# psmyth94/mamba-clip

Hardware: AMD Instinct MI355X
Metric: image-text pairs/sec (whole node) + selective_scan HBM GB/s (higher is better)
Workload: dtype bf16; 1 GPU; C2: ViT-B/16 image + Mamba-130M text, contrastive train step (fwd+bwd+AdamW), amp_bf16; model=vit_b16-mamba130m, global_batch=256, per_gpu_batch=256, seq_len=77, image_size=224, input=resident, step_launch=eager, parallelism=dp1, library_gemm_selection=tunableop-file

## Files before the change

### include/mc_gemm.h

```cpp
#ifndef MAMBA_CLIP_AMD_MC_GEMM_H
#define MAMBA_CLIP_AMD_MC_GEMM_H

#include <stddef.h>
#include <stdint.h>

#include "mc_scan.h"

#ifdef __cplusplus
extern "C" {
#endif

#define MC_WGRAD_TOKEN_MAJOR 0
#define MC_WGRAD_FEATURE_MAJOR 1

typedef struct mc_wgrad_params {
  int32_t M, N, T;
  int32_t dtype;
  int32_t a_layout, b_layout;
  const void* A;
  int64_t lda;
  const void* B;
  int64_t ldb;
  float* C;
  int64_t ldc;
  int32_t splits;
  int32_t reserved;
  void* workspace;
  size_t workspace_bytes;
} mc_wgrad_params;

size_t mc_gemm_wgrad_workspace_bytes(const mc_wgrad_params* p);
int mc_gemm_wgrad(const mc_wgrad_params* p, void* stream);

#define MC_LINEAR_EPI_NONE 0
#define MC_LINEAR_EPI_BIAS 1
#define MC_LINEAR_EPI_BIAS_GELU 2
#define MC_LINEAR_EPI_GELU_GRAD 3

typedef struct mc_linear_params {
  int32_t rows, cols, K;
  int32_t dtype;
  int32_t epilogue;
  int32_t reserved;
  const void* X; int64_t ldx;
  const void* W; int64_t ldw;
  void* Y; int64_t ldy;
  void* Y2; int64_t ldy2;
  const void* bias;
  const void* H; int64_t ldh;
  float* colsum;
  void* workspace;
  size_t workspace_bytes;
} mc_linear_params;

size_t mc_linear_workspace_bytes(const mc_linear_params* p);
int mc_linear(const mc_linear_params* p, void* stream);

int mc_gemm_small_k(int32_t M, int32_t K, int32_t T, int32_t dtype, const void* W, int64_t ldw, const void* X,
                    int64_t ldx, void* Y, int64_t ldy, void* stream);

int mc_gemm_skinny_m(int32_t M, int32_t K, int32_t T, int32_t dtype, const void* W, int64_t ldw, const void* X,
                     int64_t ldx, void* Y, int64_t ldy, void* stream);

#ifdef __cplusplus
}
#endif

#endif
```

### mamba-clip_amd/csrc/ops.hip

```cpp
#include <algorithm>

#include "mc_common.h"
#include "../../include/mc_ops.h"

namespace mc {
namespace ops {

constexpr int kMaxVec = 8;

template <int V>
__device__ __forceinline__ void ld_f32v(const float* __restrict__ p, float (&v)[V]) {
#pragma unroll
  for (int e4 = 0; e4 < V; e4 += 4) {
    const float4 q = *reinterpret_cast<const float4*>(p + e4);
    v[e4] = q.x; v[e4 + 1] = q.y; v[e4 + 2] = q.z; v[e4 + 3] = q.w;
  }
}
template <int V>
__device__ __forceinline__ void st_f32v(float* __restrict__ p, const float (&v)[V]) {
#pragma unroll
  for (int e4 = 0; e4 < V; e4 += 4)
    *reinterpret_cast<float4*>(p + e4) = make_float4(v[e4], v[e4 + 1], v[e4 + 2], v[e4 + 3]);
}

// ... 1337 lines not shown
__global__ __launch_bounds__(256) void adamw_kernel(const mc_adamw_chunk* __restrict__ chunks,
                                                    const mc_adamw_tensor* __restrict__ tensors, const mc_adamw_hyper hy) {
  const mc_adamw_chunk c = chunks[blockIdx.x];
  const mc_adamw_tensor t = tensors[c.tensor];
  const mc_adamw_group h = hy.group[c.group];
  float* __restrict__ p = t.p + c.off;
  float* __restrict__ m = t.m + c.off;
  float* __restrict__ v = t.v + c.off;
  const float* __restrict__ g = t.g + c.off;
  const bool vec = ((reinterpret_cast<uintptr_t>(p) | reinterpret_cast<uintptr_t>(m) | reinterpret_cast<uintptr_t>(v) |
                     reinterpret_cast<uintptr_t>(g)) & 15) == 0;
  const int64_t n4 = vec ? c.n / 4 : 0;
  for (int64_t i = threadIdx.x; i < n4; i += 256) {
    float4 pp = reinterpret_cast<float4*>(p)[i], mm = reinterpret_cast<float4*>(m)[i];
    float4 vv = reinterpret_cast<float4*>(v)[i];
    const float4 gg = reinterpret_cast<const float4*>(g)[i];
    adamw_elem(pp.x, mm.x, vv.x, gg.x, h);
    adamw_elem(pp.y, mm.y, vv.y, gg.y, h);
    adamw_elem(pp.z, mm.z, vv.z, gg.z, h);
    adamw_elem(pp.w, mm.w, vv.w, gg.w, h);
    reinterpret_cast<float4*>(p)[i] = pp;
    reinterpret_cast<float4*>(m)[i] = mm;
    reinterpret_cast<float4*>(v)[i] = vv;
  }
  for (int64_t i = 4 * n4 + threadIdx.x; i < c.n; i += 256) {
    float pp = p[i], mm = m[i], vv = v[i];
    adamw_elem(pp, mm, vv, g[i], h);
    p[i] = pp;
    m[i] = mm;
    v[i] = vv;
  }
}
}

extern "C" int mc_adamw_step(int32_t n_chunks, const mc_adamw_chunk* chunks, const mc_adamw_tensor* tensors,
                             const mc_adamw_hyper* hyper, void* stream) {
  MC_CHECK(n_chunks >= 0 && hyper, MC_ERR_INVALID, "mc_adamw_step: bad arguments");
  MC_CHECK(hyper->n_groups >= 1 && hyper->n_groups <= MC_ADAMW_MAX_GROUPS, MC_ERR_INVALID,
           "mc_adamw_step: n_groups %d (1..%d)", hyper->n_groups, MC_ADAMW_MAX_GROUPS);
  if (n_chunks == 0) return MC_OK;
  MC_CHECK(chunks && tensors, MC_ERR_INVALID, "mc_adamw_step: null chunk / tensor table");
  hipLaunchKernelGGL(adamw_kernel, dim3(n_chunks), dim3(256), 0, (hipStream_t)stream, chunks, tensors, *hyper);
  return check_launch("mc_adamw_step");
}

namespace {
template <bool kVec>
__global__ __launch_bounds__(256) void sum_slabs_kernel(int s, int64_t n, const float* __restrict__ src, int64_t stride,
                                                        float* __restrict__ dst) {
  const int64_t i0 = ((int64_t)blockIdx.x * 256 + threadIdx.x) * (kVec ? 4 : 1);
  if (i0 >= n) return;
  if constexpr (kVec) {
    float4 acc = *reinterpret_cast<const float4*>(src + i0);
    for (int k = 1; k < s; ++k) {
      const float4 v = *reinterpret_cast<const float4*>(src + (int64_t)k * stride + i0);
      acc.x += v.x; acc.y += v.y; acc.z += v.z; acc.w += v.w;
    }
    *reinterpret_cast<float4*>(dst + i0) = acc;
  } else {
    float acc = src[i0];
    for (int k = 1; k < s; ++k) acc += src[(int64_t)k * stride + i0];
    dst[i0] = acc;
  }
}
}

extern "C" int mc_sum_slabs(int32_t s, int64_t n, const float* src, int64_t slab_stride, float* dst, void* stream) {
  MC_CHECK(s >= 1 && n >= 0 && slab_stride >= n, MC_ERR_SHAPE, "mc_sum_slabs: bad shape (s %d, n %lld, stride %lld)", s,
           (long long)n, (long long)slab_stride);
  if (n == 0) return MC_OK;
  MC_CHECK(src && dst, MC_ERR_INVALID, "mc_sum_slabs: null pointer");
  const bool vec = n % 4 == 0 && slab_stride % 4 == 0 && aligned16(src) && aligned16(dst);
  const int64_t items = vec ? n / 4 : n;
  const dim3 grid((unsigned)((items + 255) / 256));
  if (vec) hipLaunchKernelGGL(sum_slabs_kernel<true>, grid, dim3(256), 0, (hipStream_t)stream, s, n, src, slab_stride, dst);
  else hipLaunchKernelGGL(sum_slabs_kernel<false>, grid, dim3(256), 0, (hipStream_t)stream, s, n, src, slab_stride, dst);
  return check_launch("mc_sum_slabs");
}

static int colsum_slices(int rows) { return std::max(1, std::min(kGradSlices, (rows + 31) / 32)); }

extern "C" size_t mc_colsum_workspace_bytes(int32_t rows, int32_t cols) {
  return (size_t)colsum_slices(std::max(rows, 0)) * (size_t)std::max(cols, 0) * sizeof(float);
}

extern "C" int mc_colsum(int32_t rows, int32_t cols, int32_t dtype, const void* x, int64_t ld, float* out,
                         void* workspace, size_t workspace_bytes, void* stream) {
  MC_CHECK(dtype >= MC_DTYPE_F32 && dtype <= MC_DTYPE_F16, MC_ERR_DTYPE, "mc_colsum: bad dtype");
  MC_CHECK(rows >= 0 && cols >= 0 && ld >= cols, MC_ERR_SHAPE, "mc_colsum: bad shape (rows %d, cols %d, ld %lld)",
           rows, cols, (long long)ld);
  hipStream_t s = (hipStream_t)stream;
  if (cols == 0) return MC_OK;
  MC_CHECK(out, MC_ERR_INVALID, "mc_colsum: null output");
  if (rows == 0) {
    (void)hipMemsetAsync(out, 0, (size_t)cols * 4, s);
    return check_launch("mc_colsum");
  }
  MC_CHECK(x && workspace && workspace_bytes >= mc_colsum_workspace_bytes(rows, cols), MC_ERR_WORKSPACE,
           "mc_colsum: x and a workspace of mc_colsum_workspace_bytes required");
  float* part = reinterpret_cast<float*>(workspace);
  const int ns = colsum_slices(rows);
  const int V = dtype == MC_DTYPE_F32 ? 4 : 8;
  const bool vec = cols % V == 0 && ld % V == 0 && aligned16(x);
  MC_DISPATCH_T(dtype, {
    if (vec)
      hipLaunchKernelGGL((colsum_rows_kernel<T, ElemTraits<T>::kVec>), dim3((unsigned)((cols / V + 63) / 64), ns),
                         dim3(256), 0, s, rows, cols, (const T*)x, ld, part);
// ... 41 lines not shown
```

### mamba-clip_amd/mamba_clip_amd/_lib.py

```python
import ctypes
import os

_HERE = os.path.dirname(os.path.abspath(__file__))
LIB_PATH = os.environ.get("MAMBA_CLIP_AMD_LIB") or os.path.join(_HERE, "libmamba_clip_amd.so")

MC_DTYPE_F32, MC_DTYPE_BF16, MC_DTYPE_F16, MC_DTYPE_FP8_E4M3, MC_DTYPE_U8 = 0, 1, 2, 3, 4
MC_LAYOUT_NCHW, MC_LAYOUT_NHWC = 0, 1
MC_SCAN_CHUNK = 32
MC_SCAN_STATE_INTERVAL_FINE = 8
MC_SCAN_KERNEL_NONE, MC_SCAN_KERNEL_PAIR, MC_SCAN_KERNEL_GENERIC, MC_SCAN_KERNEL_DIRS = 0, 1, 2, 3
MC_GEMM_KERNEL_TILE, MC_GEMM_KERNEL_FP8_TILE, MC_GEMM_KERNEL_FP8_PANEL = 1, 2, 3
MC_SCAN_MAX_DSTATE = 32
MC_CAST_CHUNK = 16384

c_i32, c_i64, c_vp, c_fp = ctypes.c_int32, ctypes.c_int64, ctypes.c_void_p, ctypes.c_void_p


class ScanFwdParams(ctypes.Structure):
    _fields_ = [
        ("batch", c_i32), ("dim", c_i32), ("seqlen", c_i32), ("dstate", c_i32), ("n_groups", c_i32),
        ("itype", c_i32), ("wtype", c_i32), ("delta_softplus", c_i32),
        ("u_batch_stride", c_i64), ("u_dim_stride", c_i64),
        ("delta_batch_stride", c_i64), ("delta_dim_stride", c_i64),
        ("z_batch_stride", c_i64), ("z_dim_stride", c_i64),
# ... 170 lines not shown
class SS2DMergeBwdParams(ctypes.Structure):
    _fields_ = [
        ("fwd", SS2DMergeParams), ("dy", c_vp),
        ("dy_batch_stride", c_i64), ("dy_row_stride", c_i64), ("dy_col_stride", c_i64),
        ("dout", c_fp), ("dz", c_vp), ("dln_weight", c_fp), ("dln_bias", c_fp),
        ("workspace", c_vp), ("workspace_bytes", ctypes.c_size_t),
    ]


MC_WGRAD_TOKEN_MAJOR, MC_WGRAD_FEATURE_MAJOR = 0, 1


class WgradParams(ctypes.Structure):
    _fields_ = [
        ("M", c_i32), ("N", c_i32), ("T", c_i32), ("dtype", c_i32), ("a_layout", c_i32), ("b_layout", c_i32),
        ("A", c_vp), ("lda", c_i64), ("B", c_vp), ("ldb", c_i64), ("C", c_vp), ("ldc", c_i64),
        ("splits", c_i32), ("reserved", c_i32), ("workspace", c_vp), ("workspace_bytes", ctypes.c_size_t),
    ]


MC_LINEAR_EPI_NONE, MC_LINEAR_EPI_BIAS, MC_LINEAR_EPI_BIAS_GELU, MC_LINEAR_EPI_GELU_GRAD = 0, 1, 2, 3


class LinearParams(ctypes.Structure):
    _fields_ = [
        ("rows", c_i32), ("cols", c_i32), ("K", c_i32), ("dtype", c_i32), ("epilogue", c_i32), ("reserved", c_i32),
        ("X", c_vp), ("ldx", c_i64), ("W", c_vp), ("ldw", c_i64), ("Y", c_vp), ("ldy", c_i64),
        ("Y2", c_vp), ("ldy2", c_i64), ("bias", c_vp), ("H", c_vp), ("ldh", c_i64), ("colsum", c_vp),
        ("workspace", c_vp), ("workspace_bytes", ctypes.c_size_t),
    ]


class PatchInputParams(ctypes.Structure):
    _fields_ = [
        ("batch", c_i32), ("channels", c_i32), ("height", c_i32), ("width", c_i32), ("patch", c_i32),
        ("layout", c_i32), ("in_dtype", c_i32), ("out_dtype", c_i32),
        ("img", c_vp), ("scale", c_fp), ("shift", c_fp), ("out", c_vp),
    ]


SYMBOLS = {
    "mc_last_error": (ctypes.c_char_p, []),
    "mc_version": (ctypes.c_char_p, []),
    "mc_scan_n_chunks": (c_i32, [c_i32]),
    "mc_scan_n_states": (c_i32, [c_i32, c_i32]),
    "mc_scan_fwd_state_interval": (c_i32, [ctypes.POINTER(ScanFwdParams)]),
    "mc_scan_fwd_kernel": (c_i32, [ctypes.POINTER(ScanFwdParams)]),
    "mc_gemm_wgrad_workspace_bytes": (ctypes.c_size_t, [ctypes.POINTER(WgradParams)]),
    "mc_gemm_wgrad": (ctypes.c_int, [ctypes.POINTER(WgradParams), c_vp]),
    "mc_linear_workspace_bytes": (ctypes.c_size_t, [ctypes.POINTER(LinearParams)]),
    "mc_linear": (ctypes.c_int, [ctypes.POINTER(LinearParams), c_vp]),
    "mc_gemm_small_k": (ctypes.c_int, [c_i32, c_i32, c_i32, c_i32, c_vp, c_i64, c_vp, c_i64, c_vp, c_i64, c_vp]),
    "mc_gemm_skinny_m": (ctypes.c_int, [c_i32, c_i32, c_i32, c_i32, c_vp, c_i64, c_vp, c_i64, c_vp, c_i64, c_vp]),
    "mc_scan_bwd_kernel": (c_i32, [ctypes.POINTER(ScanBwdParams)]),
    "mc_scan_chunk_states_bytes": (ctypes.c_size_t, [c_i32, c_i32, c_i32, c_i32]),
    "mc_scan_fwd_workspace_bytes": (ctypes.c_size_t, [c_i32, c_i32, c_i32, c_i32]),
    "mc_scan_bwd_workspace_bytes": (ctypes.c_size_t, [c_i32, c_i32, c_i32, c_i32, c_i32]),
    "mc_scan_fwd": (ctypes.c_int, [ctypes.POINTER(ScanFwdParams), c_vp]),
    "mc_scan_bwd": (ctypes.c_int, [ctypes.POINTER(ScanBwdParams), c_vp]),
    "mc_gemm_nt": (ctypes.c_int, [ctypes.POINTER(GemmNTParams), c_vp]),
    "mc_gemm_nt_kernel": (c_i32, [ctypes.POINTER(GemmNTParams)]),
    "mc_quant_rows_fp8": (ctypes.c_int, [c_i32, c_i32, c_i32, c_vp, c_i64, c_vp, c_i64, c_fp, c_vp]),
    "mc_ce_stats": (ctypes.c_int, [c_i32, c_i32, c_fp, c_i64, c_i32, c_i64, c_fp, c_fp, ctypes.c_float, c_fp,
                                   c_vp, ctypes.c_size_t, c_vp]),
    "mc_ce_stats_workspace_bytes": (ctypes.c_size_t, [c_i32, c_i32, c_i32]),
    "mc_ce_grad": (ctypes.c_int, [c_i32, c_i32, c_fp, c_i64, c_fp, c_i64, ctypes.c_float, c_fp, c_i64,
                                  ctypes.c_float, c_fp, c_i32, c_vp, c_i64, c_fp, c_fp, c_vp, ctypes.c_size_t, c_vp]),
    "mc_ce_grad_workspace_bytes": (ctypes.c_size_t, [c_i32, c_i32]),
    "mc_ce_fused_fwd": (ctypes.c_int, [ctypes.POINTER(CEFusedParams), c_vp]),
    "mc_ce_fused_fwd_workspace_bytes": (ctypes.c_size_t, [c_i32, c_i32, c_i32]),
    "mc_ce_fused_grad": (ctypes.c_int, [ctypes.POINTER(CEFusedParams), c_vp]),
    "mc_ce_fused_grad_workspace_bytes": (ctypes.c_size_t, [c_i32, c_i32]),
    "mc_add_rmsnorm_fwd": (ctypes.c_int, [c_i32, c_i32, c_i32, c_vp, c_fp, c_fp, ctypes.c_float, c_vp, c_fp, c_fp,
                                          c_vp]),
    "mc_add_rmsnorm_bwd": (ctypes.c_int, [c_i32, c_i32, c_i32, c_vp, c_fp, c_fp, c_fp, c_fp, c_vp, c_fp, c_fp, c_vp,
                                          ctypes.c_size_t, c_vp]),
    "mc_add_rmsnorm_bwd_workspace_bytes": (ctypes.c_size_t, [c_i32, c_i32]),
    "mc_add_layernorm_fwd": (ctypes.c_int, [c_i32, c_i32, c_i32, c_vp, c_vp, c_fp, c_fp, ctypes.c_float, c_vp, c_vp,
                                            c_fp, c_fp, c_vp]),
    "mc_add_layernorm_bwd": (ctypes.c_int, [c_i32, c_i32, c_i32, c_vp, c_vp, c_vp, c_fp, c_fp, c_fp, c_vp, c_fp, c_fp,
                                            c_fp, c_vp, ctypes.c_size_t, c_vp]),
    "mc_add_layernorm_bwd_workspace_bytes": (ctypes.c_size_t, [c_i32, c_i32]),
    "mc_causal_conv1d_fwd": (ctypes.c_int, [c_i32, c_i32, c_i32, c_i32, c_i32, c_vp, c_i64, c_i64, c_fp, c_fp, c_i32,
                                            c_vp, c_i64, c_i64, c_vp]),
    "mc_causal_conv1d_bwd": (ctypes.c_int, [c_i32, c_i32, c_i32, c_i32, c_i32, c_vp, c_i64, c_i64, c_fp, c_fp, c_i32,
                                            c_vp, c_i64, c_i64, c_vp, c_i64, c_i64, c_fp, c_fp, c_vp,
                                            ctypes.c_size_t, c_vp]),
    "mc_causal_conv1d_bwd_workspace_bytes": (ctypes.c_size_t, [c_i32, c_i32, c_i32, c_i32]),
    "mc_patch_im2col": (ctypes.c_int, [c_i32, c_i32, c_i32, c_i32, c_i32, c_i32, c_vp, c_vp, c_vp]),
    "mc_grad_colsum_workspace_bytes": (ctypes.c_size_t, [c_i32, c_i32]),
    "mc_gelu_bwd": (ctypes.c_int, [c_i32, c_i32, c_i32, c_vp, c_i64, c_vp, c_i64, c_vp, c_i64, c_fp, c_vp,
                                   ctypes.c_size_t, c_vp]),
    "mc_qkv_grad_pack": (ctypes.c_int, [ctypes.POINTER(QkvPackParams), c_vp]),
    "mc_stream_copy": (ctypes.c_int, [c_vp, c_vp, ctypes.c_size_t, c_vp]),
    "mc_cast_f32_many": (ctypes.c_int, [c_i32, c_vp, c_vp, c_i32, c_vp]),
    "mc_cast_transpose_f32_many": (ctypes.c_int, [c_i32, c_vp, c_vp, c_i32, c_vp]),
    "mc_adamw_step": (ctypes.c_int, [c_i32, c_vp, c_vp, ctypes.POINTER(AdamWHyper), c_vp]),
    "mc_sum_slabs": (ctypes.c_int, [c_i32, c_i64, c_fp, c_i64, c_fp, c_vp]),
    "mc_colsum_workspace_bytes": (ctypes.c_size_t, [c_i32, c_i32]),
    "mc_colsum_fold": (ctypes.c_int, [c_i32, c_i32, c_fp, c_fp, c_vp]),
    "mc_colsum": (ctypes.c_int, [c_i32, c_i32, c_i32, c_vp, c_i64, c_fp, c_vp, ctypes.c_size_t, c_vp]),
    "mc_l2norm_fwd": (ctypes.c_int, [c_i32, c_i32, c_i32, c_vp, c_i64, ctypes.c_float, c_fp, c_i64, c_fp, c_vp]),
    "mc_l2norm_bwd": (ctypes.c_int, [c_i32, c_i32, c_i32, c_vp, c_i64, c_fp, ctypes.c_float, c_fp, c_i64, c_vp,
                                     c_i64, c_vp]),
    "mc_attn_fwd": (ctypes.c_int, [ctypes.POINTER(AttnFwdParams), c_vp]),
    "mc_attn_bwd": (ctypes.c_int, [ctypes.POINTER(AttnBwdParams), c_vp]),
# ... 58 lines not shown
```

### mamba-clip_amd/mamba_clip_amd/ops.py

```python
import ctypes
import os
import weakref

import torch

from . import _lib


def _ws(nbytes, device):
    return torch.empty(max(int(nbytes), 16), dtype=torch.uint8, device=device)


def gemm_nt(A, B, alpha=1.0, alpha_dev=None, out_dtype=torch.float32, scale_a=None, scale_b=None, out=None):
    lib = _lib.load()
    if A.dtype != B.dtype or A.dtype not in (torch.bfloat16, torch.float32, torch.float8_e4m3fn):
        raise RuntimeError("gemm_nt: A and B must both be bf16, both fp32 or both float8_e4m3fn")
    if A.stride(-1) != 1:
        A = A.contiguous()
    if B.stride(-1) != 1:
        B = B.contiguous()
    M, K = A.shape
    N, K2 = B.shape
    if K != K2:
        raise RuntimeError("gemm_nt: inner dimensions differ")
# ... 518 lines not shown
def patch_im2col(img, patch, out_dtype=None, mean=None, std=None):
    return PatchIm2colFn.apply(img, patch, out_dtype, mean, std)


def _split_factor(M, N, K):
    if N * K >= 2_000_000:
        s = 4
    elif N * K < 250_000 or M >= 40_000:
        s = 16
    else:
        s = 8
    while s > 1 and M % s:
        s //= 2
    return s


def _wgrad_layout(t, rows_are_tokens):
    st_tok, st_feat = (t.stride(0), t.stride(1)) if rows_are_tokens else (t.stride(1), t.stride(0))
    if st_feat == 1 and t.shape[1 if rows_are_tokens else 0] > 0:
        return _lib.MC_WGRAD_TOKEN_MAJOR, st_tok
    if st_tok == 1:
        return _lib.MC_WGRAD_FEATURE_MAJOR, st_feat
    return None


def wgrad_hip(G, X, splits=0):
    if not (G.is_cuda and G.dtype == X.dtype and G.dtype in (torch.bfloat16, torch.float16)):
        return None
    N, T = G.shape
    K = X.shape[1]
    la, lb = _wgrad_layout(G, False), _wgrad_layout(X, True)
    if la is None or lb is None or T % 64 or T == 0 or G.data_ptr() % 16 or X.data_ptr() % 16:
        return None
    if la[1] % 8 or lb[1] % 8 or (la[0] == _lib.MC_WGRAD_TOKEN_MAJOR and N % 8) or \
            (lb[0] == _lib.MC_WGRAD_TOKEN_MAJOR and K % 8):
        return None
    out = torch.empty(N, K, device=G.device, dtype=torch.float32)
    p = _lib.WgradParams()
    p.M, p.N, p.T, p.dtype = N, K, T, _lib.dtype_code(G.dtype)
    p.a_layout, p.lda, p.b_layout, p.ldb = la[0], la[1], lb[0], lb[1]
    p.A, p.B, p.C, p.ldc, p.splits = G.data_ptr(), X.data_ptr(), out.data_ptr(), K, int(splits)
    lib = _lib.load()
    ws_b = lib.mc_gemm_wgrad_workspace_bytes(ctypes.byref(p))
    ws = _ws(ws_b, G.device) if ws_b else None
    if ws is not None:
        p.workspace, p.workspace_bytes = ws.data_ptr(), ws_b
    _lib.check(lib.mc_gemm_wgrad(ctypes.byref(p), _lib.stream_handle(G.device)), "mc_gemm_wgrad")
    return out


WGRAD_HIP = os.environ.get("MAMBA_CLIP_AMD_WGRAD_HIP", "1") != "0"


def wgrad(G, X):
    N, M = G.shape
    K = X.shape[1]
    if WGRAD_HIP and G.is_cuda and M >= 8192 and min(N, K) >= 256:
        out = wgrad_hip(G, X)
        if out is not None:
            return out
    s = _split_factor(M, N, K) if (G.is_cuda and M >= 8192) else 1
    if s == 1:
        return torch.mm(G, X).float()
    Gs = G.unflatten(1, (s, M // s)).transpose(0, 1)
    Xs = X.unflatten(0, (s, M // s))
    part = torch.bmm(Gs, Xs, out_dtype=torch.float32).contiguous()
    out = torch.empty(N, K, device=part.device, dtype=torch.float32)
    _lib.check(_lib.load().mc_sum_slabs(s, N * K, part.data_ptr(), part.stride(0), out.data_ptr(),
                                        _lib.stream_handle(part.device)), "mc_sum_slabs")
    return out


def colsum(x):
    if x.stride(-1) != 1:
        x = x.contiguous()
    R, C = x.shape
    out = torch.empty(C, device=x.device, dtype=torch.float32)
    lib = _lib.load()
    ws_b = lib.mc_colsum_workspace_bytes(R, C)
    ws = _ws(ws_b, x.device)
    _lib.check(lib.mc_colsum(R, C, _lib.dtype_code(x.dtype), x.data_ptr(), x.stride(0), out.data_ptr(), ws.data_ptr(),
                             ws_b, _lib.stream_handle(x.device)), "mc_colsum")
    return out


class L2NormalizeFn(torch.autograd.Function):

    @staticmethod
    def forward(ctx, x, eps):
        x2 = x if x.stride(-1) == 1 else x.contiguous()
        R, C = x2.shape
        y = torch.empty(R, C, device=x.device, dtype=torch.float32)
        norm = torch.empty(R, device=x.device, dtype=torch.float32)
        _lib.check(_lib.load().mc_l2norm_fwd(R, C, _lib.dtype_code(x2.dtype), x2.data_ptr(), x2.stride(0), eps,
                                             y.data_ptr(), C, norm.data_ptr(), _lib.stream_handle(x.device)),
                   "mc_l2norm_fwd")
        ctx.save_for_backward(x2, norm)
        ctx.eps = eps
        return y

    @staticmethod
    def backward(ctx, g):
        x2, norm = ctx.saved_tensors
        g = g.float()
        if g.stride(-1) != 1:
            g = g.contiguous()
        R, C = x2.shape
        dx = torch.empty(R, C, device=x2.device, dtype=x2.dtype)
        _lib.check(_lib.load().mc_l2norm_bwd(R, C, _lib.dtype_code(x2.dtype), x2.data_ptr(), x2.stride(0),
                                             norm.data_ptr(), ctx.eps, g.data_ptr(), g.stride(0), dx.data_ptr(), C,
                                             _lib.stream_handle(x2.device)), "mc_l2norm_bwd")
        return dx, None

# ... 292 lines not shown
                db = pre[0]
            elif g2.is_cuda:
                db = colsum(g2)
            else:
                db = torch.sum(g2, 0, dtype=torch.float32)
        return dx, dw, db


def linear_sk(x, weight, bias=None):
    return LinearSK.apply(x, weight, bias)


SMALL_K_HIP = os.environ.get("MAMBA_CLIP_AMD_SMALL_K_HIP", "1") != "0"


def small_k_ok(wc, Xc):
    K = wc.shape[1]
    return (SMALL_K_HIP and Xc.is_cuda and wc.dtype == Xc.dtype and Xc.dtype in (torch.bfloat16, torch.float16)
            and K in (16, 32, 48, 64) and Xc.shape[1] % 8 == 0 and Xc.stride(1) == 1 and Xc.stride(0) % 8 == 0
            and Xc.data_ptr() % 16 == 0 and wc.stride(1) == 1 and wc.stride(0) % 4 == 0 and wc.data_ptr() % 8 == 0)


def gemm_small_k(wc, Xc):
    M, K = wc.shape
    T = Xc.shape[1]
    y = torch.empty(M, T, device=Xc.device, dtype=Xc.dtype)
    _lib.check(_lib.load().mc_gemm_small_k(M, K, T, _lib.dtype_code(Xc.dtype), wc.data_ptr(), wc.stride(0),
                                           Xc.data_ptr(), Xc.stride(0), y.data_ptr(), T,
                                           _lib.stream_handle(Xc.device)), "mc_gemm_small_k")
    return y


SKINNY_M_HIP = os.environ.get("MAMBA_CLIP_AMD_SKINNY_M_HIP", "0") == "1"


def skinny_m_ok(wc, Xc):
    M, K = wc.shape
    return (SKINNY_M_HIP and Xc.is_cuda and wc.dtype == Xc.dtype and Xc.dtype in (torch.bfloat16, torch.float16)
            and 0 < M <= 96 and K % 256 == 0 and Xc.shape[1] % 8 == 0 and Xc.stride(1) == 1
            and Xc.stride(0) % 8 == 0 and Xc.data_ptr() % 16 == 0 and wc.stride(1) == 1 and wc.stride(0) % 4 == 0
            and wc.data_ptr() % 8 == 0)


def gemm_skinny_m(wc, Xc):
    M, K = wc.shape
    T = Xc.shape[1]
    y = torch.empty(M, T, device=Xc.device, dtype=Xc.dtype)
    _lib.check(_lib.load().mc_gemm_skinny_m(M, K, T, _lib.dtype_code(Xc.dtype), wc.data_ptr(), wc.stride(0),
                                            Xc.data_ptr(), Xc.stride(0), y.data_ptr(), T,
                                            _lib.stream_handle(Xc.device)), "mc_gemm_skinny_m")
    return y


class WeightLeftMM(torch.autograd.Function):

    @staticmethod
    def forward(ctx, weight, X, handoff=None, out_slab=None):
        dt = _compute_dtype(X)
        wc, Xc = _wcast(weight, dt), X.to(dt)
        with torch.autocast("cuda", enabled=False):
            if small_k_ok(wc, Xc):
                y = gemm_small_k(wc, Xc)
            elif skinny_m_ok(wc, Xc):
                y = gemm_skinny_m(wc, Xc)
            else:
                y = torch.mm(wc, Xc)
        ctx.save_for_backward(wc, Xc)
        ctx.handoff = handoff
        ctx.out_slab = out_slab
        return y

    @staticmethod
    def backward(ctx, gy):
        wc, Xc = ctx.saved_tensors
        g = gy.to(wc.dtype)
        dw = dX = None
        if ctx.needs_input_grad[0]:
            dw = wgrad(g, Xc.t())
        acc = ctx.handoff.take() if ctx.handoff is not None else None
        if ctx.needs_input_grad[1]:
            accv = acc.transpose(0, 1) if (acc is not None and Xc.is_contiguous()) else None
            accv = accv.view(Xc.shape) if (accv is not None and accv.is_contiguous()
                                           and accv.numel() == Xc.numel()) else None
            if accv is not None:
                dX = accv
                dX.addmm_(wc.t(), g)
                acc = None
            elif Xc.stride(0) == 1 and Xc.stride(1) != 1:
                dX = torch.mm(g.t(), wc).t()
            elif ctx.out_slab is not None and acc is None and Xc.is_contiguous():
                slab, r0 = ctx.out_slab
                dX = slab.get()[r0:r0 + Xc.shape[0]]
                torch.mm(wc.t(), g, out=dX)
            else:
                dX = torch.mm(wc.t(), g)
            if acc is not None:
                dX = dX + acc.transpose(0, 1).reshape(Xc.shape)
        return dw, dX, None, None


def wleft_mm(weight, X, handoff=None, out_slab=None):
    return WeightLeftMM.apply(weight, X, handoff, out_slab)


def mixer_proj_ok(x_cm, rank, dstate):
    dt = _compute_dtype(x_cm)
    D, T = x_cm.shape
    return (x_cm.is_cuda and dt in (torch.bfloat16, torch.float16) and x_cm.stride(1) == 1 and D % 64 == 0
            and T % 8 == 0 and T > 0 and rank % 16 == 0 and 16 <= rank <= 96 and dstate == 16
            and x_cm.stride(0) % 8 == 0 and x_cm.data_ptr() % 16 == 0)


class MixerProjFn(torch.autograd.Function):

    @staticmethod
    def forward(ctx, x, w_x, w_dt, handoff):
        dt = _compute_dtype(x)
        lib = _lib.load()
        xc = x if x.dtype == dt else x.to(dt)
        wx, wdt = _wcast(w_x, dt).contiguous(), _wcast(w_dt, dt).contiguous()
        D, T = xc.shape
        P, R = wx.shape[0], wdt.shape[1]
        xd = torch.empty(P, T, device=xc.device, dtype=dt)
        delta = torch.empty(D, T, device=xc.device, dtype=dt)
        p = _lib.MixerProjParams()
        p.dim, p.tokens, p.rank, p.proj_rows, p.dtype = D, T, R, P, _lib.dtype_code(dt)
        p.x_ld, p.x_dbl_ld, p.delta_ld = xc.stride(0), T, T
        p.x, p.w_x, p.w_dt, p.x_dbl, p.delta = xc.data_ptr(), wx.data_ptr(), wdt.data_ptr(), xd.data_ptr(), delta.data_ptr()
        _lib.check(lib.mc_mixer_proj_fwd(ctypes.byref(p), _lib.stream_handle(xc.device)), "mc_mixer_proj_fwd")
        ctx.save_for_backward(xc, wx, wdt, xd)
        ctx.handoff = handoff
        return xd[R:P - 16], xd[P - 16:], delta

    @staticmethod
    def backward(ctx, g_b, g_c, g_delta):
        xc, wx, wdt, xd = ctx.saved_tensors
        lib = _lib.load()
        D, T = xc.shape
        P, R = wx.shape[0], wdt.shape[1]
# ... 575 lines not shown
```

Before: 3721 image-text pairs/sec.

## Add skinny-wgrad and small-K accumulate HIP kernels for Mamba x_proj backward

Adds a split-token MFMA wgrad kernel for weight gradients where one dimension is at most 48 rows, used in place of bmm plus slab-sum for the long-token skinny case. Also adds a small-K backward dX GEMM that fuses the accumulation into an existing buffer, replacing addmm_ when shapes qualify, and unrolls the slab-sum loop by eight to expose more loads in flight. These target the Mamba dt/B/C projection backward, where rocBLAS handles skinny shapes poorly. The cost is new custom kernels with their own edge-case handling, plus a workspace for the partial sums.

```diff
diff --git a/include/mc_gemm.h b/include/mc_gemm.h
--- a/include/mc_gemm.h
+++ b/include/mc_gemm.h
@@ -62,6 +62,13 @@
 int mc_gemm_skinny_m(int32_t M, int32_t K, int32_t T, int32_t dtype, const void* W, int64_t ldw, const void* X,
                      int64_t ldx, void* Y, int64_t ldy, void* stream);
 
+int mc_gemm_small_k_acc(int32_t M, int32_t K, int32_t T, int32_t dtype, const void* Wk, int64_t ldw, const void* X,
+                        int64_t ldx, const void* Z, int64_t ldz, void* Y, int64_t ldy, void* stream);
+
+size_t mc_wgrad_skinny_workspace_bytes(int32_t R, int32_t D, int32_t T);
+int mc_wgrad_skinny(int32_t R, int32_t D, int32_t T, int32_t dtype, const void* S, int64_t lds, const void* Wd,
+                    int64_t ldw, int32_t wide_major, float* C, void* workspace, size_t workspace_bytes, void* stream);
+
 #ifdef __cplusplus
 }
 #endif
diff --git a/mamba-clip_amd/csrc/gemm_skinny.hip b/mamba-clip_amd/csrc/gemm_skinny.hip
--- /dev/null
+++ b/mamba-clip_amd/csrc/gemm_skinny.hip
@@ -0,0 +1,312 @@
+#include <algorithm>
+#include <type_traits>
+
+#include "mc_common.h"
+#include "../../include/mc_gemm.h"
+
+extern "C" int mc_sum_slabs(int32_t s, int64_t n, const float* src, int64_t slab_stride, float* dst, void* stream);
+
+namespace mc {
+namespace skinny_wgrad {
+constexpr int kWD = 128;
+constexpr int kTok = 128;
+constexpr int kRow = 272;
+constexpr int kTargetWG = 256;
+constexpr int kPD = 4;
+
+typedef __bf16 bf16x8 __attribute__((ext_vector_type(8)));
+typedef _Float16 f16x8 __attribute__((ext_vector_type(8)));
+
+template <typename T>
+__device__ __forceinline__ f32x4 mfma32(const uint4& a, const uint4& b, const f32x4& c) {
+  if constexpr (std::is_same<T, bf16_t>::value)
+    return __builtin_amdgcn_mfma_f32_16x16x32_bf16(__builtin_bit_cast(bf16x8, a), __builtin_bit_cast(bf16x8, b), c, 0, 0, 0);
+  else
+    return __builtin_amdgcn_mfma_f32_16x16x32_f16(__builtin_bit_cast(f16x8, a), __builtin_bit_cast(f16x8, b), c, 0, 0, 0);
+}
+
+template <typename T, int NB>
+__global__ __launch_bounds__(256) void wgrad_skinny_kernel(int R, int D, int Tn, int chunks_per, int dblocks,
+                                                           const T* __restrict__ S, int64_t lds_,
+                                                           const T* __restrict__ Wd, int64_t ldw,
+                                                           float* __restrict__ P, int64_t slab, int wide_major) {
+  __shared__ __attribute__((aligned(16))) char sm[2][NB * 16 * kRow];
+  const int tid = threadIdx.x, lane = tid & 63, w = tid >> 6;
+  const int g = lane >> 4, i = lane & 15;
+  const int db = blockIdx.x % dblocks, rg = blockIdx.x / dblocks;
+  const int d0 = db * kWD + 32 * w;
+  const int nchunks = (Tn + kTok - 1) / kTok;
+  const int c0 = rg * chunks_per, c1 = min(nchunks, c0 + chunks_per);
+  int64_t wrow[2];
+#pragma unroll
+  for (int rb = 0; rb < 2; ++rb) wrow[rb] = (int64_t)min(d0 + 16 * rb + i, D - 1) * ldw;
+  struct Bundle { uint4 w[2][4]; uint4 s[NB]; };
+  Bundle q[kPD];
+  auto keep = [](bool ok, const uint4& v) __attribute__((always_inline)) {
+    return make_uint4(ok ? v.x : 0u, ok ? v.y : 0u, ok ? v.z : 0u, ok ? v.w : 0u);
+  };
+  const int sr = tid >> 4, st = (tid & 15) * 8;
+  auto load = [&](int c, Bundle& b) __attribute__((always_inline)) {
+    const int t0 = c * kTok;
+    const bool live = c < c1;
+#pragma unroll
+    for (int rb = 0; rb < 2; ++rb)
+#pragma unroll
+      for (int s = 0; s < 4; ++s) {
+        const int t = t0 + 32 * s + 8 * g;
+        b.w[rb][s] = ld16(Wd + ((live & (t < Tn)) ? wrow[rb] + t : (int64_t)0));
+      }
+#pragma unroll
+    for (int j = 0; j < NB; ++j) {
+      const int r = sr + 16 * j, t = t0 + st;
+      b.s[j] = ld16(S + ((live & (r < R) & (t < Tn)) ? (int64_t)r * lds_ + t : (int64_t)0));
+    }
+  };
+  f32x4 acc[2][NB];
+#pragma unroll
+  for (int rb = 0; rb < 2; ++rb)
+#pragma unroll
+    for (int nb = 0; nb < NB; ++nb) acc[rb][nb] = f32x4{0.f, 0.f, 0.f, 0.f};
+#pragma unroll
+  for (int d = 0; d < kPD; ++d) load(c0 + d, q[d]);
+  int c = c0;
+  auto step = [&](Bundle& b) __attribute__((always_inline)) {
+    char* img = sm[(c - c0) & 1];
+    const int t0 = c * kTok;
+#pragma unroll
+    for (int j = 0; j < NB; ++j)
+      *reinterpret_cast<uint4*>(img + (sr + 16 * j) * kRow + st * 2) = keep(sr + 16 * j < R && t0 + st < Tn, b.s[j]);
+    __syncthreads();
+    uint4 n[4][NB];
+#pragma unroll
+    for (int s = 0; s < 4; ++s)
+#pragma unroll
+      for (int nb = 0; nb < NB; ++nb)
+        n[s][nb] = *reinterpret_cast<const uint4*>(img + (16 * nb + i) * kRow + 64 * s + 16 * g);
+    __builtin_amdgcn_sched_barrier(0);
+#pragma unroll
+    for (int s = 0; s < 4; ++s)
+#pragma unroll
+      for (int nb = 0; nb < NB; ++nb)
+#pragma unroll
+        for (int rb = 0; rb < 2; ++rb) acc[rb][nb] = mfma32<T>(b.w[rb][s], n[s][nb], acc[rb][nb]);
+    load(c + kPD, b);
+  };
+  static_assert(kPD == 4, "the rotation below is written out for four slots");
+  for (;;) {
+    step(q[0]); if (++c >= c1) break;
+    step(q[1]); if (++c >= c1) break;
+    step(q[2]); if (++c >= c1) break;
+    step(q[3]); if (++c >= c1) break;
+  }
+  float* out = P + (int64_t)rg * slab;
+#pragma unroll
+  for (int rb = 0; rb < 2; ++rb)
+#pragma unroll
+    for (int nb = 0; nb < NB; ++nb) {
+      const int r = 16 * nb + i, d = d0 + 16 * rb + 4 * g;
+      if (r >= R) continue;
+      const f32x4 v = acc[rb][nb];
+      if (wide_major) {
+#pragma unroll
+        for (int j = 0; j < 4; ++j)
+          if (d + j < D) out[(int64_t)(d + j) * R + r] = v[j];
+      } else if ((D & 3) == 0) {
+        if (d < D) *reinterpret_cast<f32x4*>(out + (int64_t)r * D + d) = v;
+      } else {
+#pragma unroll
+        for (int j = 0; j < 4; ++j)
+          if (d + j < D) out[(int64_t)r * D + d + j] = v[j];
+      }
+    }
+}
+
+struct Split { int dblocks, chunks_per, ranges; };
+static Split split_of(int D, int T) {
+  Split s;
+  s.dblocks = (D + kWD - 1) / kWD;
+  const int nchunks = (T + kTok - 1) / kTok;
+  const int target = std::max(1, std::min(nchunks, kTargetWG / std::max(1, s.dblocks)));
+  s.chunks_per = (nchunks + target - 1) / target;
+  s.ranges = (nchunks + s.chunks_per - 1) / s.chunks_per;
+  return s;
+}
+static bool shape_ok(int R, int D, int T) { return R > 0 && R <= 96 && D > 0 && T > 0 && T % 8 == 0; }
+}
+}
+
+using namespace mc;
+
+extern "C" size_t mc_wgrad_skinny_workspace_bytes(int32_t R, int32_t D, int32_t T) {
+  if (!skinny_wgrad::shape_ok(R, D, T)) return 0;
+  const skinny_wgrad::Split s = skinny_wgrad::split_of(D, T);
+  return s.ranges > 1 ? (size_t)s.ranges * (size_t)R * (size_t)D * sizeof(float) : 0;
+}
+
+extern "C" int mc_wgrad_skinny(int32_t R, int32_t D, int32_t T, int32_t dtype, const void* S, int64_t lds_,
+                               const void* Wd, int64_t ldw, int32_t wide_major, float* C, void* workspace,
+                               size_t workspace_bytes, void* stream) {
+  MC_CHECK(dtype == MC_DTYPE_BF16 || dtype == MC_DTYPE_F16, MC_ERR_DTYPE, "mc_wgrad_skinny: bf16 / f16 only");
+  MC_CHECK(skinny_wgrad::shape_ok(R, D, T), MC_ERR_SHAPE, "mc_wgrad_skinny: 0 < R %d <= 96, D %d > 0, T %d > 0, T %% 8 == 0",
+           R, D, T);
+  MC_CHECK(S && Wd && C && aligned16(S) && aligned16(Wd) && aligned16(C) && lds_ % 8 == 0 && lds_ >= T && ldw % 8 == 0 &&
+               ldw >= T,
+           MC_ERR_SHAPE, "mc_wgrad_skinny: 16-B aligned operand rows (ld %% 8 == 0, ld >= T) and output");
+  const skinny_wgrad::Split sp = skinny_wgrad::split_of(D, T);
+  const size_t need = mc_wgrad_skinny_workspace_bytes(R, D, T);
+  MC_CHECK(need == 0 || (workspace && aligned16(workspace) && workspace_bytes >= need), MC_ERR_WORKSPACE,
+           "mc_wgrad_skinny: a 16-B aligned workspace of mc_wgrad_skinny_workspace_bytes (%zu B) required", need);
+  float* P = sp.ranges > 1 ? reinterpret_cast<float*>(workspace) : C;
+  const int64_t slab = (int64_t)R * D;
+  const dim3 grid((unsigned)(sp.dblocks * sp.ranges)), block(256);
+  hipStream_t s = (hipStream_t)stream;
+  const int nb = (R + 15) / 16, wm = wide_major ? 1 : 0;
+#define MC_WSK(TT, NBV) hipLaunchKernelGGL((skinny_wgrad::wgrad_skinny_kernel<TT, NBV>), grid, block, 0, s, R, D, T, \
+                                           sp.chunks_per, sp.dblocks, (const TT*)S, lds_, (const TT*)Wd, ldw, P, slab, wm)
+#define MC_WSK_T(TT) \
+  switch (nb) { case 1: MC_WSK(TT, 1); break; case 2: MC_WSK(TT, 2); break; case 3: MC_WSK(TT, 3); break; \
+                case 4: MC_WSK(TT, 4); break; case 5: MC_WSK(TT, 5); break; default: MC_WSK(TT, 6); break; }
+  if (dtype == MC_DTYPE_BF16) { MC_WSK_T(bf16_t) } else { MC_WSK_T(f16_t) }
+#undef MC_WSK_T
+#undef MC_WSK
+  hipError_t e = hipGetLastError();
+  MC_CHECK(e == hipSuccess, MC_ERR_LAUNCH, "mc_wgrad_skinny: launch failed: %s", hipGetErrorString(e));
+  if (sp.ranges > 1) return mc_sum_slabs(sp.ranges, slab, P, slab, C, stream);
+  return MC_OK;
+}
+
+namespace mc {
+namespace skinny_acc {
+constexpr int kTT = 256, kTM = 64, kRow = 544, kORow = 528, kWRow = 136;
+typedef short s16x4_t __attribute__((ext_vector_type(4)));
+typedef __attribute__((address_space(3))) s16x4_t lds_s16x4_t;
+
+template <typename T>
+__device__ __forceinline__ f32x4 mfma16(s16x4_t a, s16x4_t b, f32x4 c) {
+  if constexpr (std::is_same<T, bf16_t>::value) return __builtin_amdgcn_mfma_f32_16x16x16bf16_1k(a, b, c, 0, 0, 0);
+  else {
+    typedef _Float16 h4 __attribute__((ext_vector_type(4)));
+    return __builtin_amdgcn_mfma_f32_16x16x16f16(__builtin_bit_cast(h4, a), __builtin_bit_cast(h4, b), c, 0, 0, 0);
+  }
+}
+
+__device__ __forceinline__ s16x4_t tr_read(const char* base, int off) {
+  return __builtin_amdgcn_ds_read_tr16_b64_v4i16((lds_s16x4_t*)((__attribute__((address_space(3))) char*)(base) + off));
+}
+
+template <typename T, int K, bool kZ>
+__global__ __launch_bounds__(256) void small_k_acc_kernel(int M, int Tn, const T* __restrict__ Wk, int64_t ldw,
+                                                          const T* __restrict__ X, int64_t ldx, const T* Z,
+                                                          int64_t ldz, T* Y, int64_t ldy) {
+  constexpr int kXs = K * kRow > kTM * kORow ? K * kRow : kTM * kORow;
+  __shared__ __attribute__((aligned(16))) char xs[kXs + K * kWRow];
+  char* ws = xs + kXs;
+  const int tid = threadIdx.x, lane = tid & 63, w = tid >> 6;
+  const int tiles_t = (Tn + kTT - 1) / kTT;
+  const int t0 = (blockIdx.x % tiles_t) * kTT, m0 = (blockIdx.x / tiles_t) * kTM;
+  constexpr int kVecs = K * kTT / 8;
+#pragma unroll
+  for (int j = 0; j < (kVecs + 255) / 256; ++j) {
+    const int v = tid + 256 * j;
+    if (v < kVecs) {
+      const int r = v / (kTT / 8), c = (v % (kTT / 8)) * 8;
+      uint4 x = make_uint4(0u, 0u, 0u, 0u);
+      if (t0 + c < Tn) x = ld16(X + (int64_t)r * ldx + t0 + c);
+      *reinterpret_cast<uint4*>(xs + r * kRow + c * 2) = x;
+    }
+  }
+  constexpr int kPieces = K * (kTM / 4);
+#pragma unroll
+  for (int j = 0; j < (kPieces + 255) / 256; ++j) {
+    const int v = tid + 256 * j;
+    if (v < kPieces) {
+      const int r = v >> 4, c = (v & 15) * 4;
+      uint2 x = make_uint2(0u, 0u);
+      if (m0 + c < M) x = *reinterpret_cast<const uint2*>(Wk + (int64_t)r * ldw + m0 + c);
+      *reinterpret_cast<uint2*>(ws + r * kWRow + c * 2) = x;
+    }
+  }
+  const int cv = tid & 31, rr = tid >> 5;
+  uint4 zr[kTM / 8];
+  if constexpr (kZ) {
+#pragma unroll
+    for (int j = 0; j < kTM / 8; ++j) {
+      const int m = m0 + 8 * j + rr, t = t0 + cv * 8;
+      zr[j] = (m < M && t < Tn) ? ld16(Z + (int64_t)m * ldz + t) : make_uint4(0u, 0u, 0u, 0u);
+    }
+  }
+  __syncthreads();
+  const int g = lane >> 4, i = lane & 15, q = i >> 2, p = i & 3;
+  s16x4_t bfr[4][K / 16];
+#pragma unroll
+  for (int cb = 0; cb < 4; ++cb)
+#pragma unroll
+    for (int kk = 0; kk < K / 16; ++kk) bfr[cb][kk] = tr_read(ws, (16 * kk + 4 * g + q) * kWRow + (16 * cb + 4 * p) * 2);
+  f32x4 acc[4][4];
+#pragma unroll
+  for (int tb = 0; tb < 4; ++tb)
+#pragma unroll
+    for (int cb = 0; cb < 4; ++cb) acc[tb][cb] = f32x4{0.f, 0.f, 0.f, 0.f};
+#pragma unroll
+  for (int kk = 0; kk < K / 16; ++kk)
+#pragma unroll
+    for (int tb = 0; tb < 4; ++tb) {
+      const s16x4_t a = tr_read(xs, (16 * kk + 4 * g + q) * kRow + (w * 64 + tb * 16 + 4 * p) * 2);
+#pragma unroll
+      for (int cb = 0; cb < 4; ++cb) acc[tb][cb] = mfma16<T>(a, bfr[cb][kk], acc[tb][cb]);
+    }
+  __syncthreads();
+  if constexpr (kZ) {
+#pragma unroll
+    for (int j = 0; j < kTM / 8; ++j) *reinterpret_cast<uint4*>(xs + (8 * j + rr) * kORow + cv * 16) = zr[j];
+    __syncthreads();
+  }
+#pragma unroll
+  for (int tb = 0; tb < 4; ++tb)
+#pragma unroll
+    for (int cb = 0; cb < 4; ++cb) {
+      f32x4 v = acc[tb][cb];
+      uint2* slot = reinterpret_cast<uint2*>(xs + (16 * cb + i) * kORow + (w * 64 + tb * 16 + 4 * g) * 2);
+      if constexpr (kZ) {
+        typedef T t4 __attribute__((ext_vector_type(4)));
+        v += __builtin_convertvector(__builtin_bit_cast(t4, *slot), f32x4);
+      }
+      *slot = make_uint2(cvt_pk2<T>(v[0], v[1]), cvt_pk2<T>(v[2], v[3]));
+    }
+  __syncthreads();
+#pragma unroll
+  for (int j = 0; j < kTM / 8; ++j) {
+    const int r = 8 * j + rr, m = m0 + r, t = t0 + cv * 8;
+    if (m < M && t < Tn) st16(Y + (int64_t)m * ldy + t, *reinterpret_cast<const uint4*>(xs + r * kORow + cv * 16));
+  }
+}
+}
+}
+
+extern "C" int mc_gemm_small_k_acc(int32_t M, int32_t K, int32_t T, int32_t dtype, const void* Wk, int64_t ldw,
+                                   const void* X, int64_t ldx, const void* Z, int64_t ldz, void* Y, int64_t ldy,
+                                   void* stream) {
+  MC_CHECK(dtype == MC_DTYPE_BF16 || dtype == MC_DTYPE_F16, MC_ERR_DTYPE, "mc_gemm_small_k_acc: bf16 / f16 only");
+  MC_CHECK(M > 0 && M % 4 == 0 && K >= 16 && K <= 96 && K % 16 == 0 && T >= 0 && T % 8 == 0, MC_ERR_SHAPE,
+           "mc_gemm_small_k_acc: M %d > 0, M %% 4 == 0, K %d %% 16 == 0 in [16, 96], T %d %% 8 == 0", M, K, T);
+  MC_CHECK(Wk && X && Y && aligned16(X) && aligned16(Y) && (reinterpret_cast<uintptr_t>(Wk) & 7) == 0 && ldw % 4 == 0 &&
+               ldw >= M && ldx % 8 == 0 && ldx >= T && ldy % 8 == 0 && ldy >= T,
+           MC_ERR_SHAPE, "mc_gemm_small_k_acc: 16-B aligned X / Y rows (ld %% 8), 8-B aligned Wk rows (ldw %% 4, >= M)");
+  MC_CHECK(!Z || (aligned16(Z) && ldz % 8 == 0 && ldz >= T), MC_ERR_SHAPE,
+           "mc_gemm_small_k_acc: 16-B aligned Z rows (ldz %% 8, >= T)");
+  if (T == 0) return MC_OK;
+  const dim3 grid(((T + skinny_acc::kTT - 1) / skinny_acc::kTT) * ((M + skinny_acc::kTM - 1) / skinny_acc::kTM)), block(256);
+  hipStream_t s = (hipStream_t)stream;
+#define MC_SKA(TT, KK, ZZ) hipLaunchKernelGGL((skinny_acc::small_k_acc_kernel<TT, KK, ZZ>), grid, block, 0, s, M, T, \
+                                              (const TT*)Wk, ldw, (const TT*)X, ldx, (const TT*)Z, ldz, (TT*)Y, ldy)
+#define MC_SKA_K(TT, ZZ) \
+  switch (K) { case 16: MC_SKA(TT, 16, ZZ); break; case 32: MC_SKA(TT, 32, ZZ); break; case 48: MC_SKA(TT, 48, ZZ); break; \
+               case 64: MC_SKA(TT, 64, ZZ); break; case 80: MC_SKA(TT, 80, ZZ); break; default: MC_SKA(TT, 96, ZZ); break; }
+  if (dtype == MC_DTYPE_BF16) { if (Z) { MC_SKA_K(bf16_t, true) } else { MC_SKA_K(bf16_t, false) } }
+  else { if (Z) { MC_SKA_K(f16_t, true) } else { MC_SKA_K(f16_t, false) } }
+#undef MC_SKA_K
+#undef MC_SKA
+  hipError_t e = hipGetLastError();
+  MC_CHECK(e == hipSuccess, MC_ERR_LAUNCH, "mc_gemm_small_k_acc: launch failed: %s", hipGetErrorString(e));
+  return MC_OK;
+}
diff --git a/mamba-clip_amd/csrc/ops.hip b/mamba-clip_amd/csrc/ops.hip
--- a/mamba-clip_amd/csrc/ops.hip
+++ b/mamba-clip_amd/csrc/ops.hip
@@ -1413,7 +1413,15 @@
   if (i0 >= n) return;
   if constexpr (kVec) {
     float4 acc = *reinterpret_cast<const float4*>(src + i0);
-    for (int k = 1; k < s; ++k) {
+    int k = 1;
+    for (; k + 8 <= s; k += 8) {
+      float4 v[8];
+#pragma unroll
+      for (int j = 0; j < 8; ++j) v[j] = *reinterpret_cast<const float4*>(src + (int64_t)(k + j) * stride + i0);
+#pragma unroll
+      for (int j = 0; j < 8; ++j) { acc.x += v[j].x; acc.y += v[j].y; acc.z += v[j].z; acc.w += v[j].w; }
+    }
+    for (; k < s; ++k) {
       const float4 v = *reinterpret_cast<const float4*>(src + (int64_t)k * stride + i0);
       acc.x += v.x; acc.y += v.y; acc.z += v.z; acc.w += v.w;
     }
diff --git a/mamba-clip_amd/mamba_clip_amd/_lib.py b/mamba-clip_amd/mamba_clip_amd/_lib.py
--- a/mamba-clip_amd/mamba_clip_amd/_lib.py
+++ b/mamba-clip_amd/mamba_clip_amd/_lib.py
@@ -246,6 +246,11 @@
     "mc_linear": (ctypes.c_int, [ctypes.POINTER(LinearParams), c_vp]),
     "mc_gemm_small_k": (ctypes.c_int, [c_i32, c_i32, c_i32, c_i32, c_vp, c_i64, c_vp, c_i64, c_vp, c_i64, c_vp]),
     "mc_gemm_skinny_m": (ctypes.c_int, [c_i32, c_i32, c_i32, c_i32, c_vp, c_i64, c_vp, c_i64, c_vp, c_i64, c_vp]),
+    "mc_gemm_small_k_acc": (ctypes.c_int, [c_i32, c_i32, c_i32, c_i32, c_vp, c_i64, c_vp, c_i64, c_vp, c_i64, c_vp,
+                                           c_i64, c_vp]),
+    "mc_wgrad_skinny_workspace_bytes": (ctypes.c_size_t, [c_i32, c_i32, c_i32]),
+    "mc_wgrad_skinny": (ctypes.c_int, [c_i32, c_i32, c_i32, c_i32, c_vp, c_i64, c_vp, c_i64, c_i32, c_fp, c_vp,
+                                       ctypes.c_size_t, c_vp]),
     "mc_scan_bwd_kernel": (c_i32, [ctypes.POINTER(ScanBwdParams)]),
     "mc_scan_chunk_states_bytes": (ctypes.c_size_t, [c_i32, c_i32, c_i32, c_i32]),
     "mc_scan_fwd_workspace_bytes": (ctypes.c_size_t, [c_i32, c_i32, c_i32, c_i32]),
diff --git a/mamba-clip_amd/mamba_clip_amd/ops.py b/mamba-clip_amd/mamba_clip_amd/ops.py
--- a/mamba-clip_amd/mamba_clip_amd/ops.py
+++ b/mamba-clip_amd/mamba_clip_amd/ops.py
@@ -594,6 +594,36 @@
 WGRAD_HIP = os.environ.get("MAMBA_CLIP_AMD_WGRAD_HIP", "1") != "0"
 
 
+WGRAD_SKINNY_HIP = os.environ.get("MAMBA_CLIP_AMD_WGRAD_SKINNY_HIP", "1") != "0"
+WGRAD_SKINNY_MAX_ROWS = int(os.environ.get("MAMBA_CLIP_AMD_WGRAD_SKINNY_MAX_ROWS", "48"))
+
+
+def wgrad_skinny_ok(G, X):
+    N, T = G.shape
+    K = X.shape[1]
+    return (WGRAD_SKINNY_HIP and G.is_cuda and G.dtype == X.dtype and G.dtype in (torch.bfloat16, torch.float16)
+            and 0 < min(N, K) <= min(96, WGRAD_SKINNY_MAX_ROWS) and T > 0 and T % 8 == 0
+            and G.stride(1) == 1 and X.stride(0) == 1 and G.stride(0) % 8 == 0 and X.stride(1) % 8 == 0
+            and G.stride(0) >= T and X.stride(1) >= T and G.data_ptr() % 16 == 0 and X.data_ptr() % 16 == 0)
+
+
+def wgrad_skinny(G, X):
+    N, T = G.shape
+    K = X.shape[1]
+    out = torch.empty(N, K, device=G.device, dtype=torch.float32)
+    lib = _lib.load()
+    if N <= 96:
+        R, D, S, lds, Wd, ldw, wide_major = N, K, G, G.stride(0), X, X.stride(1), 0
+    else:
+        R, D, S, lds, Wd, ldw, wide_major = K, N, X, X.stride(1), G, G.stride(0), 1
+    ws_b = lib.mc_wgrad_skinny_workspace_bytes(R, D, T)
+    ws = _ws(ws_b, G.device) if ws_b else None
+    _lib.check(lib.mc_wgrad_skinny(R, D, T, _lib.dtype_code(G.dtype), S.data_ptr(), lds, Wd.data_ptr(), ldw,
+                                   wide_major, out.data_ptr(), ws.data_ptr() if ws is not None else None, ws_b,
+                                   _lib.stream_handle(G.device)), "mc_wgrad_skinny")
+    return out
+
+
 def wgrad(G, X):
     N, M = G.shape
     K = X.shape[1]
@@ -601,6 +631,8 @@
         out = wgrad_hip(G, X)
         if out is not None:
             return out
+    if G.is_cuda and M >= 8192 and wgrad_skinny_ok(G, X):
+        return wgrad_skinny(G, X)
     s = _split_factor(M, N, K) if (G.is_cuda and M >= 8192) else 1
     if s == 1:
         return torch.mm(G, X).float()
@@ -999,6 +1031,32 @@
     return y
 
 
+SMALL_K_ACC_HIP = os.environ.get("MAMBA_CLIP_AMD_SMALL_K_ACC_HIP", "1") != "0"
+
+
+def small_k_acc_ok(wc, g, Z=None):
+    K, M = wc.shape
+    T = g.shape[1]
+    return (SMALL_K_ACC_HIP and g.is_cuda and wc.dtype == g.dtype and g.dtype in (torch.bfloat16, torch.float16)
+            and g.shape[0] == K and K % 16 == 0 and 16 <= K <= 96 and M > 0 and M % 4 == 0 and T % 8 == 0
+            and wc.stride(1) == 1 and wc.stride(0) % 4 == 0 and wc.stride(0) >= M and wc.data_ptr() % 8 == 0
+            and g.stride(1) == 1 and g.stride(0) % 8 == 0 and g.stride(0) >= T and g.data_ptr() % 16 == 0
+            and (Z is None or (Z.dtype == g.dtype and Z.shape == (M, T) and Z.stride(1) == 1 and Z.stride(0) % 8 == 0
+                               and Z.stride(0) >= T and Z.data_ptr() % 16 == 0)))
+
+
+def gemm_small_k_acc(wc, g, Z=None, out=None):
+    K, M = wc.shape
+    T = g.shape[1]
+    if out is None:
+        out = torch.empty(M, T, device=g.device, dtype=g.dtype)
+    _lib.check(_lib.load().mc_gemm_small_k_acc(M, K, T, _lib.dtype_code(g.dtype), wc.data_ptr(), wc.stride(0),
+                                               g.data_ptr(), g.stride(0), Z.data_ptr() if Z is not None else None,
+                                               Z.stride(0) if Z is not None else 0, out.data_ptr(), out.stride(0),
+                                               _lib.stream_handle(g.device)), "mc_gemm_small_k_acc")
+    return out
+
+
 class WeightLeftMM(torch.autograd.Function):
 
     @staticmethod
@@ -1031,7 +1089,10 @@
                                            and accv.numel() == Xc.numel()) else None
             if accv is not None:
                 dX = accv
-                dX.addmm_(wc.t(), g)
+                if small_k_acc_ok(wc, g, dX):
+                    gemm_small_k_acc(wc, g, dX, dX)
+                else:
+                    dX.addmm_(wc.t(), g)
                 acc = None
             elif Xc.stride(0) == 1 and Xc.stride(1) != 1:
                 dX = torch.mm(g.t(), wc).t()
```

Result: no change. 3740 image-text pairs/sec (median of 6 runs) (+0.5%).
